# aluo-x/3D_SLN

Hardware: AMD Instinct MI355X
Metric: scene-graph VAE steps/sec + 256² diff-render fps, 1/2/4/8 MI355X (higher is better)
Workload: dtype f32; 1 GPU; BASELINE configs[1]: batch=64 scene graphs x (32 objects, 64 triples) per GPU, Sg2ScVAE train step at train.py defaults (embedding_dim=64, 5+5 GraphTripleConv, BatchNorm); O=2048, T=4096, hipgraph=True, distinct_batches_cycled=4, eps=N(0,1) drawn on the device inside the step, parallelism=dp1

## Files before the change

3d_sln_amd/_lib.py:

```python
from __future__ import annotations

import ctypes as C
import os

HERE = os.path.dirname(os.path.abspath(__file__))
LIB_PATH = os.path.join(HERE, "libsln_hip.so")

SLN_E = {-1: "SLN_E_BADARG", -2: "SLN_E_UNSUPPORTED", -3: "SLN_E_STATE", -4: "SLN_E_NOGPU", -5: "SLN_E_NOMEM", -6: "SLN_E_CAPTURE"}

c_f32p = C.c_void_p
c_i64p = C.c_void_p


class SlnError(RuntimeError):
    pass


class SlnVaeConfig(C.Structure):
    _fields_ = [(n, C.c_int) for n in (
        "embedding_dim", "gconv_num_layers", "recurrent", "batch_norm", "decoder_cat", "use_ae",
        "box_dim", "n_angle", "num_objs", "num_preds", "num_attrs", "no_attr")]


class SlnVaeUnit(C.Structure):
# ... 189 lines not shown
    "sln_debug_gemm_nt": (C.c_int, [C.POINTER(SlnDbgGemmNT), C.c_int, C.POINTER(C.c_int), C.c_void_p]),
    "sln_debug_gemm_tn": (C.c_int, [C.POINTER(SlnDbgGemmTN), C.c_int, C.c_int, C.c_void_p]),
    "sln_debug_gemm_nt_route": (C.c_int, [C.POINTER(SlnDbgGemmNT), C.POINTER(SlnDbgNTRoute)]),
    "sln_debug_gemm_nt_half": (C.c_int, [C.POINTER(SlnDbgGemmNT), C.c_int, C.c_void_p]),
    "sln_debug_gemm_nt_half_takes": (C.c_int, [C.POINTER(SlnDbgGemmNT)]),
    "sln_debug_gemm_sizes": (C.c_int, [C.POINTER(C.c_int), C.c_int]),
    "sln_debug_vae_csr": (C.c_int, [c_i64p, C.c_int, C.c_int, C.c_int, C.POINTER(SlnDbgCsr), C.c_void_p, C.c_void_p]),
    "sln_debug_vae_edge": (C.c_int, [C.POINTER(SlnDbgEdge), C.c_int, C.c_int, C.POINTER(C.c_int), C.c_void_p]),
    "sln_debug_vae_loss": (C.c_int, [C.POINTER(SlnDbgLoss), C.c_void_p]),
    "sln_debug_vae_tables": (C.c_int, [C.c_int, C.c_void_p, C.c_int, C.c_int, C.c_float, C.c_int, C.c_int, C.c_int, C.c_void_p]),
    "sln_debug_vae_embed": (C.c_int, [C.POINTER(SlnDbgEmbed), C.c_int, C.c_int, C.POINTER(C.c_int), C.c_void_p]),
    "sln_debug_vae_opt": (C.c_int, [C.POINTER(SlnDbgOpt), C.c_void_p]),
    "sln_debug_vae_sizes": (C.c_int, [C.POINTER(C.c_int), C.c_int]),
    "sln_debug_vae_leaf_launches": (C.c_int64, [C.c_void_p]),
    "sln_debug_vae_half_launches": (C.c_int64, [C.c_void_p]),
    "sln_project_faces": (C.c_int, [c_f32p, C.c_void_p, c_f32p, c_f32p, c_f32p, C.c_int, C.c_int, C.c_int, C.c_float, C.c_float, c_f32p, C.c_void_p]),
    "sln_project_faces_backward": (C.c_int, [c_f32p, C.c_void_p, c_f32p, c_f32p, c_f32p, C.c_int, C.c_int, C.c_int, C.c_float, C.c_float, c_f32p,
                                             c_f32p, C.c_void_p]),
    "sln_raster_workspace_bytes": (C.c_int64, [C.c_int, C.c_int]),
    "sln_raster_forward": (C.c_int, [c_f32p, C.c_int, C.c_int, C.c_int, C.c_float, C.c_float, C.c_void_p, C.c_void_p,
                                     c_f32p, c_f32p, C.c_void_p]),
    "sln_raster_forward_dual": (C.c_int, [c_f32p, C.c_int, C.c_int, C.c_int, C.c_float, C.c_float, C.c_float, C.c_void_p,
                                          C.c_void_p, c_f32p, c_f32p, C.c_void_p, c_f32p, c_f32p, C.c_void_p]),
    "sln_raster_texture_sample": (C.c_int, [c_f32p, c_f32p, C.c_void_p, c_f32p, c_f32p, C.c_int, C.c_int, C.c_int, C.c_int,
                                            C.c_float, c_f32p, C.c_void_p]),
    "sln_raster_backward_depth": (C.c_int, [c_f32p, C.c_void_p, c_f32p, c_f32p, c_f32p, C.c_int, C.c_int, C.c_int, c_f32p,
                                            C.c_void_p]),
    "sln_raster_backward_rgb": (C.c_int, [c_f32p, C.c_void_p, c_f32p, c_f32p, C.c_int, C.c_int, C.c_int, C.c_int, C.c_float,
                                          c_f32p, C.c_void_p]),
    "sln_raster_texture_sample_chw": (C.c_int, [c_f32p, c_f32p, C.c_void_p, c_f32p, c_f32p, C.c_int, C.c_int, C.c_int, C.c_int, C.c_int,
# ... 138 lines not shown
```

3d_sln_amd/csrc/sln_debug.h:

```cpp
#pragma once
#include "sln_common.h"
#include "sln_hip.h"

bool sln_dbg_bn(const SlnDbgBn& d, int coef, BnView& v);
long sln_vae_engine_leaf_launches(const SlnVae* h);
long sln_vae_engine_half_launches(const SlnVae* h);
```

3d_sln_amd/csrc/vae_debug.hip:

```cpp
#include <cstdint>
#include <cstring>
#include <vector>
#include "sln_debug.h"
#include "vae_multi.h"

namespace {

bool dbg_csr(const SlnDbgCsr& d, GraphCsr& g) {
  std::memset(&g, 0, sizeof(g));
  if (d.T < 0 || d.O < 1 || !d.deg || !d.invdeg || !d.rowptr || !d.cursor) return false;
  if (d.T > 0 && (!d.s || !d.p || !d.o || !d.ent)) return false;
  g.s = d.s; g.p = d.p; g.o = d.o; g.deg = d.deg; g.invdeg = d.invdeg; g.rowptr = d.rowptr; g.cursor = d.cursor; g.ent = d.ent;
  g.T = d.T; g.O = d.O;
  return true;
}

bool dbg_fwd_bn(const SlnDbgBn& d, int cols, BnView& v) {
  if (!sln_dbg_bn(d, SLN_COEF_FWD, v)) return false;
  return d.mode != SLN_BN_TRAIN || d.cstride >= cols;
}

enum { E_SCATTER_FWD = 0, E_SCATTER_BWD = 1, E_GATHER_BWD = 2, E_MASK_GSTATS = 3, E_BN_RELU = 4, E_ADD2 = 5 };

bool dbg_edge_ok(const SlnDbgEdge& d, GraphCsr& g, BnView& bn) {
// ... 150 lines not shown

extern "C" int sln_debug_vae_sizes(int* out, int max) {
  const int sz[7] = {(int)sizeof(SlnDbgCsr), (int)sizeof(SlnDbgEdge), (int)sizeof(SlnDbgLoss), (int)sizeof(SlnDbgBnEntry),
                     (int)sizeof(SlnDbgTranspose), (int)sizeof(SlnDbgOpt), (int)sizeof(SlnDbgEmbed)};
  for (int i = 0; out && i < 7 && i < max; ++i) out[i] = sz[i];
  return 7;
}

extern "C" int sln_debug_vae_csr(const int64_t* triples, int num_preds, int edges_only, int deg_is_zero, const SlnDbgCsr* desc, int* err,
                                 void* stream) {
  GraphCsr g;
  if (!desc || !dbg_csr(*desc, g) || (g.T > 0 && !triples) || (!edges_only && num_preds < 1)) return SLN_E_BADARG;
  return sln_launch_graph_prep(triples, g.T, g.O, edges_only ? 1 : num_preds, g, err, (hipStream_t)stream, edges_only ? 1 : 0, deg_is_zero ? 1 : 0);
}

extern "C" int sln_debug_vae_edge(const SlnDbgEdge* desc, int n, int multi, int* variant, void* stream) {
  if (!desc || n < 1 || n > 64 || (!multi && n != 1)) return SLN_E_BADARG;
  hipStream_t st = (hipStream_t)stream;
  std::vector<GraphCsr> g((size_t)n);
  std::vector<BnView> bn((size_t)n);
  for (int i = 0; i < n; ++i)
    if (desc[i].kind != desc[0].kind || !dbg_edge_ok(desc[i], g[(size_t)i], bn[(size_t)i])) return SLN_E_BADARG;
  if (variant) *variant = -1;
  if (!multi) return edge_single(desc[0], g[0], bn[0], st);
  if (sln_capturing(st)) return SLN_E_CAPTURE;
  switch (desc[0].kind) {
    case E_SCATTER_FWD: {
      std::vector<MScatterFwd> rooms((size_t)n);
      for (int i = 0; i < n; ++i) { const SlnDbgEdge& d = desc[i]; rooms[(size_t)i] = MScatterFwd{d.a, d.lda, d.H, d.D, bn[(size_t)i], g[(size_t)i], d.rows, d.out, 0, 0}; }
      return edge_multi(rooms, [](MScatterFwd& m) { return sln_plan_scatter_avg_fwd(m); }, [](const MScatterFwd* t, int R, int var, int gx, int gy, hipStream_t s) { return sln_launch_scatter_avg_fwd_multi(t, R, var, gx, gy, s); }, variant, st);
// ... 167 lines not shown
  for (int k = 0; k < d->calls && !r; ++k)
    r = d->kind == 0   ? sln_launch_adam(d->params, d->grads, d->m, d->v, (long)d->n, sc.p, d->total_loss, st)
        : d->kind == 1 ? sln_launch_randn(d->params, (long)d->n, sc.p, st)
                       : sln_launch_step_prologue(pro, st);
  const int rs = (int)hipStreamSynchronize(st);
  if (!r) r = rs;
  if (!r) r = (int)hipMemcpy(h.data(), sc.p, sizeof(AdamScalars), hipMemcpyDeviceToHost);
  if (sc.p) (void)hipFree(sc.p);
  if (r) return r;
  d->out_step = h[0].step; d->out_offset = h[0].rng_offset; d->out_bc1 = h[0].bc1; d->out_bc2 = h[0].bc2; d->out_skip = h[0].skip;
  if (h[0].adam_done != 0 || h[0].rng_done != 0) return SLN_E_STATE;
  return 0;
}

extern "C" int64_t sln_debug_vae_leaf_launches(const SlnVae* h) { return h ? (int64_t)sln_vae_engine_leaf_launches(h) : (int64_t)SLN_E_BADARG; }
extern "C" int64_t sln_debug_vae_half_launches(const SlnVae* h) { return h ? (int64_t)sln_vae_engine_half_launches(h) : (int64_t)SLN_E_BADARG; }
```

3d_sln_amd/csrc/vae_engine.hip:

```cpp
#include <cstddef>
#include <new>
#include <type_traits>
#include <utility>
#include <vector>
#include <cstring>
#include <cstdlib>

#include "../../include/sln_hip.h"
#include "sln_gemm.h"
#include "vae_kernels.h"
#include "vae_multi.h"
#include "sln_prof.h"

namespace {

enum { SK_DEC_ASSEMBLE = 0, SK_EMBED_GATHER, SK_NT, SK_SCATTER_FWD, SK_TN, SK_TN_FLUSH, SK_MASK_GSTATS, SK_ADD2, SK_EMBED_BWD,
       SK_SCATTER_BWD, SK_GATHER_BWD, SK_DEC_ASSEMBLE_BWD, SK_COPY2D };
struct RecStep {
  int kind = -1, epi = 0, idx64 = 0;
  GemmNTArgs nt; GemmTNArgs tn;
  MScatterFwd sf; MScatterBwd sb; MGatherBwd gb; MMaskGstats mg; MDecAssemble da; DecAssembleBwd dab; MEmbedGather eg; MEmbedBwd eb; MAdd2 a2;
};
struct Recorder { std::vector<RecStep> steps; };

// ... 216 lines not shown
    deferred.clear();
    return 0;
  }

  hipGraphExec_t graph_exec[4] = {nullptr, nullptr, nullptr, nullptr}; int graph_O[4] = {-1, -1, -1, -1}, graph_T[4] = {-1, -1, -1, -1};

  bool it_zero_in_prologue = false;
  bool it_prologue = false;
  bool it_fused_loss = false;
  bool it_one_flush = false;
  bool one_flush = true;
  bool it_merge_bn = false;
  bool no_merge = false;
  bool it_leaf = false;
  bool it_wt_prologue = false;
  bool leaf_merge = true;
  long leaf_launches = 0;
  int gemm_precision = 0;
  bool in_iteration = false;
  long half_launches = 0;
  bool gconv_only = false;
  int unit_of(int net, int l, int k) const { return (gconv_only ? 0 : 8) + (net * nmod + (cfg.recurrent ? 0 : l)) * 4 + k; }
  int unit_boxnet(int k) const { return 8 + 2 * nmod * 4 + k; }
  int unit_anglenet(int k) const { return 8 + 2 * nmod * 4 + 2 + k; }

  int bn_mode(const BnInst& b, bool training) const {
    if (b.unit < 0 || !units[b.unit].bn) return SLN_BN_NONE;
    return training ? SLN_BN_TRAIN : SLN_BN_EVAL;
  }
  BnView view(int inst, int col0, bool training) const {
    BnView v; std::memset(&v, 0, sizeof(v));
    v.eps = kBnEps; v.n_rows = 1.f; v.rn = 1.0; v.mode = SLN_BN_NONE;
// ... 358 lines not shown

int SlnVae::encoder_forward(bool training, hipStream_t st) {
  if (training && enc_stats_doubles && !bulk_zeroed) RET_IF(sln_zero_async(stats_base, enc_stats_doubles * sizeof(double), st));
  EncAssemble ea; std::memset(&ea, 0, sizeof(ea));
  ea.objs = batch.objs; ea.attrs = batch.attributes; ea.angles = batch.angles; ea.boxes = batch.boxes;
  ea.obj_emb = t.obj_emb_ec; ea.attr_emb = t.attr_emb_ec; ea.angle_emb = t.angle_emb; ea.wb = t.box_emb_w; ea.bb = t.box_emb_b;
  ea.O = O; ea.n_obj = n_obj_e; ea.n_attr = n_attr_e; ea.n_box = n_box_e; ea.n_angle = n_angle_e; ea.box_dim = cfg.box_dim;
  ea.x0 = X0e;
  if (it_prologue) {
    StepPrologue sp; std::memset(&sp, 0, sizeof(sp));
    sp.eps = draw_eps ? eps_buf : nullptr; sp.n_eps = (long)O * E; sp.scalars = scalars;
    sp.enc = ea; sp.pidx = g.p; sp.T = T;
    sp.pemb_ec = t.pred_emb_ec; sp.n_ec = Dec; sp.p0e = P0e;
    sp.pemb_dc = t.pred_emb_dc; sp.n_dc = Ddc; sp.p0d = P0d;
    if (it_zero_in_prologue) { sp.zero_ptr = zero_begin; sp.zero_bytes = (long)zero_bytes; }
    if (it_wt_prologue && !wt_fresh) { sp.tr_tab = tr_table_dev; sp.n_tr = n_tr; sp.tr_max_tiles = tr_max_tiles; }
    RET_IF(sln_launch_step_prologue(sp, st));
    if (sp.tr_tab) wt_fresh = true;
  } else {
    RET_IF(sln_launch_enc_assemble(ea, st));
    RET_IF(sln_launch_embed_gather_i32(g.p, t.pred_emb_ec, T, Dec, P0e, st));
  }
  for (int l = 0; l < L; ++l) RET_IF(gconv_forward(l, training, st));
  const Operand XL = layer_output(L - 1, training);
  const int W = 2 * E;
  begin_group();
  RET_IF(linear_fwd(XL, 0, hbA1, H, 0, O, bn_head[0], training, st));
  RET_IF(linear_fwd(XL, 4, haA1, H, 0, O, bn_head[2], training, st));
  RET_IF(end_group(st));
  begin_group();
// ... 204 lines not shown
    int maxc = 0;
    for (auto& bi : bns) maxc = bi.C > maxc ? bi.C : maxc;
    RET_IF(sln_launch_bn_param_grads(bn_table_dev, (int)bns.size(), maxc, cfg.recurrent ? 0 : 1, st));
  } else if (n_bn_enc > 0) {
    int maxc = 0;
    for (int i = 0; i < n_bn_enc; ++i) maxc = bns[i].C > maxc ? bns[i].C : maxc;
    RET_IF(sln_launch_bn_param_grads(bn_table_dev, n_bn_enc, maxc, cfg.recurrent ? 0 : 1, st));
  }
  RET_IF(flush_deferred(it_one_flush ? 2 : 1, st));
  return 0;
}

int SlnVae::train_iteration(const float* eps, int mode, hipStream_t st) {
  int r = 0;
  if (mode != TRAIN_ENCODER_BWD) {
    HIP_RET(hipMemsetAsync(t.flat_grads, 0, sizeof(float) * (size_t)t.n_flat, st));
    const bool no_merge = this->no_merge;
    it_prologue = it_fused_loss = !no_merge;
    it_zero_in_prologue = it_prologue && (reinterpret_cast<uintptr_t>(zero_begin) & 15) == 0 && (zero_bytes & 15) == 0;
    if (!it_zero_in_prologue) HIP_RET(hipMemsetAsync(zero_begin, 0, zero_bytes, st));
    bulk_zeroed = true;
    it_merge_bn = !no_merge && (mode == TRAIN_BACKWARD || mode == TRAIN_FULL);
    it_one_flush = one_flush && !tn_per_layer && (mode == TRAIN_BACKWARD || mode == TRAIN_FULL);
    it_leaf = it_merge_bn && dG[2] != nullptr && T > 0 && sln_vae_leaf_fits(leaf_args()) != 0;
    it_wt_prologue = it_prologue && leaf_merge && (mode == TRAIN_BACKWARD || mode == TRAIN_FULL);
    if (!it_prologue && draw_eps) r = sln_launch_randn(eps_buf, (long)O * E, scalars, st);
    in_iteration = true;
    if (!r) r = encoder_forward(step_training, st);
    if (!r) r = decoder_forward(nullptr, eps, step_training, st);
    in_iteration = false;
    if (!r) r = loss(boxes_pred, angles_pred, mu, logvar, true, st);
    if (!r && grad_guard && mode != TRAIN_FULL)
      r = (int)hipMemcpyAsync(grad_guard, losses + 3, sizeof(float), hipMemcpyDeviceToDevice, st);
    if (!r) r = decoder_backward(st);
    if (!r) r = sln_launch_latent_bwd(mu, logvar, eps, dz, &scalars->kl_weight, O, E, cfg.use_ae, dmu, dlv, st);
  }
  if (mode != TRAIN_UPTO_DECODER) {
    bulk_zeroed = true;
    if (!r) r = encoder_backward(st);
  }
  bulk_zeroed = false;
  it_prologue = it_fused_loss = it_merge_bn = it_zero_in_prologue = it_one_flush = it_leaf = it_wt_prologue = false;
  RET_IF(r);
  if (mode == TRAIN_FULL) {
    RET_IF(sln_launch_adam(t.flat_params, t.flat_grads, t.adam_m, t.adam_v, (long)t.n_flat, scalars, losses + 3, st));
    wt_fresh = false;
  }
  return 0;
}

long sln_vae_engine_leaf_launches(const SlnVae* h) { return h->leaf_launches; }
long sln_vae_engine_half_launches(const SlnVae* h) { return h->half_launches; }

extern "C" {

int sln_version(void) { return 1; }
const char* sln_build_arch(void) { return "gfx950"; }
int sln_device_ok(void) {
  int n = 0;
  if (hipGetDeviceCount(&n) != hipSuccess || n <= 0) return SLN_E_NOGPU;
  hipDeviceProp_t p;
  int dev = 0;
  if (hipGetDevice(&dev) != hipSuccess || hipGetDeviceProperties(&p, dev) != hipSuccess) return SLN_E_NOGPU;
  return std::strncmp(p.gcnArchName, "gfx950", 6) == 0 ? 0 : SLN_E_NOGPU;
}

static int cfg_check(const SlnVaeConfig* c) {
// ... 6 lines not shown
}

int sln_vae_num_units(const SlnVaeConfig* c) {
  if (cfg_check(c) != 0) return cfg_check(c);
  const int nmod = c->recurrent ? 1 : c->gconv_num_layers;
  return 8 + 2 * nmod * 4 + 4;
}

static int read_engine_options(SlnVae* h) {
  auto is = [](const char* name, char c) { const char* v = std::getenv(name); return v && v[0] == c; };
  h->use_group = !is("SLN_NO_GROUP", '1');
  h->no_merge = is("SLN_NO_MERGE", '1');
  h->tn_per_layer = is("SLN_TN_PER_LAYER", '1');
  h->one_flush = !is("SLN_TN_ONE_FLUSH", '0');
  h->leaf_merge = !is("SLN_LEAF_MERGE", '0');
  h->tn_slots = 3 * (2 * h->L + 8 > 16 ? 2 * h->L + 8 : 16);
  h->tn_groups_store = new (std::nothrow) SlnVae::TnGroup[2 * (size_t)h->tn_slots * 2];
  return h->tn_groups_store ? 0 : SLN_E_BADARG;
}

int sln_vae_create(const SlnVaeConfig* c, SlnVae** out) {
  if (!out) return SLN_E_BADARG;
  int r = cfg_check(c);
  if (r != 0) return r;
  SlnVae* h = new (std::nothrow) SlnVae();
  if (!h) return SLN_E_BADARG;
  h->cfg = *c;
  const int E = c->embedding_dim;
  h->E = E; h->H = 4 * E; h->L = c->gconv_num_layers; h->nmod = c->recurrent ? 1 : h->L;
  h->n_obj_e = c->no_attr ? E : E * 3 / 4; h->n_attr_e = c->no_attr ? 0 : E / 4; h->n_box_e = E * 3 / 4; h->n_angle_e = E / 4;
// ... 116 lines not shown
    for (auto& ly : h->layers)
      for (int k = 0; k < 4; ++k)
        if (ly.bn[k] >= 0) h->bns[ly.bn[k]].rows = k < 2 ? b->T : b->O;
    for (int s = 0; s < 6; ++s)
      if (h->bn_head[s] >= 0) h->bns[h->bn_head[s]].rows = b->O;
    if (!h->bn_table_live) {
      HIP_RET(hipStreamSynchronize(st));
      RET_IF(upload_bn_table(h));
      h->bn_table_live = true;
    }
    bool has_graph = false;
    for (int i = 0; i < 4; ++i) has_graph |= h->graph_exec[i] != nullptr;
    if (has_graph) HIP_RET(hipStreamSynchronize(st));
    h->drop_graphs();
  }
  RET_IF(sln_zero_async(h->err_flag, sizeof(int), st));
  StageBatch sb; std::memset(&sb, 0, sizeof(sb));
  sb.objs = b->objs; sb.attrs = b->attributes; sb.angles = b->angles; sb.boxes = b->boxes;
  sb.st_objs = h->st_objs; sb.st_attrs = h->st_attrs; sb.st_angles = h->st_angles; sb.st_boxes = h->st_boxes;
  sb.attrs32 = h->attrs32; sb.deg = h->g.deg; sb.err = h->err_flag;
  sb.O = b->O; sb.box_dim = h->cfg.box_dim; sb.n_objs = h->cfg.num_objs; sb.n_attrs = h->cfg.num_attrs; sb.n_angle = h->cfg.n_angle;
  RET_IF(sln_launch_stage_batch(sb, st));
  h->batch.objs = h->st_objs; h->batch.angles = h->st_angles; h->batch.attributes = h->st_attrs; h->batch.boxes = h->st_boxes;
  RET_IF(sln_launch_graph_prep(b->triples, b->T, b->O, h->cfg.num_preds, h->g, h->err_flag, st, 0, 1));
  h->batch_set = true; h->have_enc = h->have_dec = false;
  return 0;
}

int sln_vae_check_batch(SlnVae* h, void* stream) {
  if (!h || !h->batch_set) return SLN_E_STATE;
  int flag = 0;
  HIP_RET(hipMemcpyAsync(&flag, h->err_flag, sizeof(int), hipMemcpyDeviceToHost, (hipStream_t)stream));
  HIP_RET(hipStreamSynchronize((hipStream_t)stream));
  return flag ? SLN_E_BADARG : 0;
}

static int copy_out(float* dst, const float* src, size_t n, hipStream_t st) {
  if (!dst || dst == src) return 0;
  return (int)hipMemcpyAsync(dst, src, n * sizeof(float), hipMemcpyDeviceToDevice, st);
// ... 844 lines not shown
```

3d_sln_amd/csrc/vae_kernels.h:

```cpp
#pragma once
#include "sln_common.h"

struct GraphCsr {
  int* s;
  int* p;
  int* o;
  int* deg;
  float* invdeg;
  int* rowptr;
  int* cursor;
  int* ent;
  int T, O;
};
int sln_launch_graph_prep(const int64_t* triples, int T, int O, int num_preds, GraphCsr g, int* err_flag, hipStream_t st,
                          int edges_only = 0, int deg_is_zero = 0);
int sln_launch_bn_relu_apply(const float* x, int ld, int col0, int cols, int rows, BnView bn, float* out, int ldo, hipStream_t st);
struct StageBatch {
  const int64_t* objs; const int64_t* attrs; const int64_t* angles; const float* boxes;
  int64_t* st_objs; int64_t* st_attrs; int64_t* st_angles; float* st_boxes;
  int* attrs32; int* deg; int* err;
  int O, box_dim, n_objs, n_attrs, n_angle;
};
int sln_launch_stage_batch(const StageBatch& a, hipStream_t st);
int sln_launch_validate_ids(const int64_t* objs, const int64_t* attrs, const int64_t* angles, int O, int n_objs, int n_attrs,
                            int n_angle, int* err_flag, hipStream_t st);

int sln_launch_scatter_avg_fwd(const float* A2, int ld, int H, int D, BnView bn2, GraphCsr g, int O,
                               float* pooled, hipStream_t st);

int sln_launch_scatter_avg_bwd(const float* dM, const float* dP, int lddp, int dpcol0, const float* A2, int ld,
                               int H, int D, BnView bn2, GraphCsr g, int T, float* g2, double* gsums,
                               int cstride, hipStream_t st);

int sln_launch_gather_bwd(const float* dG, int ldg, int D, GraphCsr g, int O, const float* add1, int ldadd1,
                          const float* xprev, int ldx, BnView bn, int masked, float* out, int ldo,
                          double* gsums, int cstride, hipStream_t st);

int sln_launch_add2(const float* a, int lda, const float* b, int ldb, int rows, int cols, float* out, int ldo, hipStream_t st);
// ... 75 lines not shown
  int64_t step; float lr, beta1, beta2, eps; float kl_weight; float bc1, bc2; int skip, pad_;
  unsigned long long rng_seed, rng_offset; unsigned int rng_done, adam_done;
};
int sln_launch_adam(float* params, const float* grads, float* m, float* v, long n, AdamScalars* scalars, const float* total_loss,
                    hipStream_t st);

int sln_launch_randn(float* eps, long n, AdamScalars* scalars, hipStream_t st);

struct StepPrologue {
  float* eps; long n_eps; AdamScalars* scalars;
  EncAssemble enc;
  const int* pidx; int T;
  const float* pemb_ec; int n_ec; float* p0e;
  const float* pemb_dc; int n_dc; float* p0d;
  void* zero_ptr; long zero_bytes;
  const TransposeEntry* tr_tab; int n_tr, tr_max_tiles;
};
int sln_launch_step_prologue(const StepPrologue& a, hipStream_t st);

struct VaeLeaf {
  EncAssembleBwd enc;
  const int* pidx; int pred_rows, pred_table_rows;
  const float* d_pdc; int ld_pdc, col0_pdc, n_pdc; float* d_pred_dc;
  const float* d_pec; int ld_pec, col0_pec, n_pec; float* d_pred_ec;
  const int64_t* attr_idx; const float* d_attr; int ld_attr, col0_attr, n_attr_dc, attr_table_rows; float* d_attr_dc;
  const BnTableEntry* bn_tab; int bn_n, bn_max_c, bn_independent;
  int bn_update; float bn_momentum;
};
int sln_vae_leaf_fits(const VaeLeaf& a);
int sln_launch_vae_leaf(const VaeLeaf& a, hipStream_t st);
// ... 2 lines not shown
```

3d_sln_amd/csrc/vae_kernels.hip:

```cpp
#include <cstring>
#include "vae_kernels.h"
#include "sln_prof.h"

namespace {

constexpr int CB = 64;
constexpr int RL = 4;
constexpr int BOX_ROWS = 64;
constexpr int RB = 32;

__device__ __forceinline__ void commit_col_stats(float s1, float s2, bool valid, double* out, int cstride, int col) {
  __shared__ float red[2][RL][CB];
  red[0][threadIdx.y][threadIdx.x] = s1;
  red[1][threadIdx.y][threadIdx.x] = s2;
  __syncthreads();
  if (threadIdx.y == 0 && valid && out != nullptr) {
    float a = 0.f, b = 0.f;
#pragma unroll
    for (int i = 0; i < RL; ++i) { a += red[0][i][threadIdx.x]; b += red[1][i][threadIdx.x]; }
    atomicAdd(out + col, sln_qd((double)a, SLN_Q_BWD));
    atomicAdd(out + cstride + col, sln_qd((double)b, SLN_Q_BWD));
  }
}

// ... 806 lines not shown
    }
#pragma unroll
    for (int k = 0; k < 4; ++k)
      if (4 * q + k < n) eps[4 * q + k] = v[k];
  }
  __syncthreads();
  if (threadIdx.x == 0) {
    const unsigned int done = atomicAdd(&sc->rng_done, 1u);
    if (done == nblocks - 1) { sc->rng_done = 0; sc->rng_offset = off + 1; }
  }
}
__global__ __launch_bounds__(256) void randn_kernel(float* __restrict__ eps, long n, AdamScalars* sc) {
  randn_body(eps, n, sc, blockIdx.x, gridDim.x);
}

__global__ __launch_bounds__(256) void step_prologue_kernel(StepPrologue a, unsigned int b0, unsigned int b1, unsigned int b2, unsigned int b3,
                                                            unsigned int b4) {
  __shared__ float tile[32][33];
  const unsigned int b = blockIdx.x;
  if (b < b0) randn_body(a.eps, a.n_eps, a.scalars, b, b0);
  else if (b < b1) enc_assemble_body(a.enc, b - b0);
  else if (b < b2) embed_gather_body(a.pidx, a.pemb_ec, a.T, a.n_ec, a.p0e, b - b1);
  else if (b < b3) embed_gather_body(a.pidx, a.pemb_dc, a.T, a.n_dc, a.p0d, b - b2);
  else if (b < b4) {
    const long i = (long)(b - b3) * 256 + threadIdx.x;
    if (i * 16 < a.zero_bytes) reinterpret_cast<uint4*>(a.zero_ptr)[i] = make_uint4(0u, 0u, 0u, 0u);
  } else {
    const unsigned int q = b - b4;
    const TransposeEntry t = a.tr_tab[q / (unsigned int)a.tr_max_tiles];
    transpose_tile_body(t, (int)(q % (unsigned int)a.tr_max_tiles), tile);
  }
}

__global__ void bn_relu_apply_kernel(const float* __restrict__ x, int ld, int col0, int cols, long n, BnView bn,
                                     float* __restrict__ out, int ldo) {
  const long i = (long)blockIdx.x * blockDim.x + threadIdx.x;
  if (i >= n) return;
  const long r = i / cols; const int c = (int)(i % cols);
  float sc, sh;
  bn_fwd_coef(bn, c, sc, sh);
  out[r * ldo + c] = fmaxf(fmaf(sc, x[r * ld + col0 + c], sh), 0.f);
}

// ... 25 lines not shown
  const int i = blockIdx.x * blockDim.x + threadIdx.x;
  if (i >= a.O) return;
  const int64_t ob = a.objs[i], at = a.attrs[i], an = a.angles[i];
  a.st_objs[i] = ob; a.st_attrs[i] = at; a.st_angles[i] = an;
  a.attrs32[i] = (int)at;
  a.deg[i] = 0;
  for (int k = 0; k < a.box_dim; ++k) a.st_boxes[(size_t)i * a.box_dim + k] = a.boxes[(size_t)i * a.box_dim + k];
  if (ob < 0 || ob >= a.n_objs) atomicOr(a.err, 2);
  if (a.n_attrs > 0 && (at < 0 || at >= a.n_attrs)) atomicOr(a.err, 4);
  if (an < 0 || an >= a.n_angle) atomicOr(a.err, 8);
}

int sln_launch_stage_batch(const StageBatch& a, hipStream_t st) {
  if (a.O <= 0) return 0;
  hipLaunchKernelGGL(stage_batch_kernel, dim3(sln_cdiv(a.O, 256)), dim3(256), 0, st, a);
  SLN_CHECK_LAUNCH();
  return 0;
}

int sln_launch_validate_ids(const int64_t* objs, const int64_t* attrs, const int64_t* angles, int O, int n_objs, int n_attrs,
                            int n_angle, int* err_flag, hipStream_t st) {
  if (O <= 0) return 0;
  hipLaunchKernelGGL(validate_ids_kernel, dim3(sln_cdiv(O, 256)), dim3(256), 0, st, objs, attrs, angles, O, n_objs, n_attrs, n_angle,
                     err_flag);
  SLN_CHECK_LAUNCH();
  return 0;
}

int sln_launch_graph_prep(const int64_t* triples, int T, int O, int num_preds, GraphCsr g, int* err_flag, hipStream_t st,
                          int edges_only, int deg_is_zero) {
// ... 360 lines not shown

int sln_launch_randn(float* eps, long n, AdamScalars* scalars, hipStream_t st) {
  if (n <= 0) return 0;
  const long q = (n + 3) / 4;
  hipLaunchKernelGGL(randn_kernel, dim3((unsigned)((q + 255) / 256)), dim3(256), 0, st, eps, n, scalars);
  SLN_CHECK_LAUNCH();
  return 0;
}

int sln_launch_step_prologue(const StepPrologue& a, hipStream_t st) {
  auto blocks = [](long n) { return (unsigned int)((n + 255) / 256); };
  const unsigned int nr = a.eps ? blocks((a.n_eps + 3) / 4) : 0;
  const unsigned int ne = blocks((long)a.enc.O * (a.enc.n_obj + a.enc.n_attr + a.enc.n_box + a.enc.n_angle));
  const unsigned int n1 = blocks((long)a.T * a.n_ec), n2 = blocks((long)a.T * a.n_dc);
  const unsigned int nz = a.zero_ptr ? blocks(a.zero_bytes / 16) : 0;
  const unsigned int nt = (a.tr_tab && a.n_tr > 0 && a.tr_max_tiles > 0) ? (unsigned int)a.n_tr * (unsigned int)a.tr_max_tiles : 0;
  const unsigned int tot = nr + ne + n1 + n2 + nz + nt;
  if (tot == 0) return 0;
  hipLaunchKernelGGL(step_prologue_kernel, dim3(tot), dim3(256), 0, st, a, nr, nr + ne, nr + ne + n1, nr + ne + n1 + n2, nr + ne + n1 + n2 + nz);
  SLN_CHECK_LAUNCH();
  return 0;
}

struct LeafEmbedJob { const void* idx; const float* d; float* d_emb; int ld, col0, rows, n, table_rows, rpb; };
struct LeafArgs {
  AssembleBwdLds asmb;
  EncAssembleBwd box; int box_gx;
  LeafEmbedJob pdc, pec, attr;
  const BnTableEntry* bn_tab; int bn_n, bn_per_entry, bn_gx, rows_t, rows_o; float mom;
};
__global__ __launch_bounds__(256) void vae_leaf_kernel(unsigned int b0, unsigned int b1, unsigned int b2, unsigned int b3, unsigned int b4,
                                                       unsigned int b5, LeafArgs a) {
  extern __shared__ float tab[];
  const unsigned int b = blockIdx.x;
// ... 354 lines not shown
```

include/sln_hip.h:

```cpp
#ifndef SLN_HIP_H
#define SLN_HIP_H

#include <stdint.h>

#ifdef __cplusplus
extern "C" {
#endif

#define SLN_E_BADARG (-1)
#define SLN_E_UNSUPPORTED (-2)
#define SLN_E_STATE (-3)
#define SLN_E_NOGPU (-4)
#define SLN_E_NOMEM (-5)
#define SLN_E_CAPTURE (-6)

int sln_version(void);
const char* sln_build_arch(void);
int sln_device_ok(void);


typedef struct SlnVaeConfig {
  int embedding_dim;
  int gconv_num_layers;
  int recurrent;
// ... 220 lines not shown
  int kind, O, n_obj, n_attr, n_box, n_angle, box_dim, n_z, use_ae, z_in_x0, rows_obj, rows_attr, rows_angle, ld, col0, n, table_rows,
      T, n2, pad_;
} SlnDbgEmbed;
int sln_debug_vae_embed(const SlnDbgEmbed* desc, int n, int multi, int* variant, void* stream);
typedef struct SlnDbgOpt {
  float* params; const float* grads; float* m; float* v; const float* total_loss; const SlnDbgEmbed* pro;
  int64_t n, step;
  uint64_t seed, offset;
  float lr, beta1, beta2, eps;
  int kind, calls;
  int64_t out_step; uint64_t out_offset; float out_bc1, out_bc2; int out_skip, pad_;
} SlnDbgOpt;
int sln_debug_vae_opt(SlnDbgOpt* desc, void* stream);
int sln_debug_vae_sizes(int* out, int max);
int64_t sln_debug_vae_leaf_launches(const SlnVae* h);
int64_t sln_debug_vae_half_launches(const SlnVae* h);


int sln_project_faces(const float* vertices, const int32_t* faces, const float* K, const float* R, const float* t, int B, int V, int F,
                      float orig_size, float eps, float* faces_xyz, void* stream);
int sln_project_faces_backward(const float* vertices, const int32_t* faces, const float* K, const float* R, const float* t, int B, int V,
                               int F, float orig_size, float eps, const float* grad_faces_xyz, float* grad_vertices, void* stream);
int64_t sln_raster_workspace_bytes(int B, int F);
int sln_raster_forward(const float* faces, int B, int F, int image_size, float near, float far, void* workspace,
                       int32_t* face_index, float* weight, float* depth, void* stream);
int sln_raster_forward_dual(const float* faces, int B, int F, int image_size, float near_a, float near_b, float far,
                            void* workspace, int32_t* fi_a, float* w_a, float* d_a, int32_t* fi_b, float* w_b,
                            float* d_b, void* stream);
int sln_raster_texture_sample(const float* faces, const float* textures, const int32_t* face_index, const float* weight,
                              const float* depth, int B, int F, int image_size, int texture_size, float eps, float* rgb,
// ... 199 lines not shown
```

Before: 35500 graphs/s (scene-graph VAE fwd+loss+bwd+Adam).

## Fuse batch staging and CSR graph prep into one kernel; merge grad clear into prologue

```diff
diff --git a/3d_sln_amd/_lib.py b/3d_sln_amd/_lib.py
--- a/3d_sln_amd/_lib.py
+++ b/3d_sln_amd/_lib.py
@@ -227,6 +227,9 @@
     "sln_debug_vae_sizes": (C.c_int, [C.POINTER(C.c_int), C.c_int]),
     "sln_debug_vae_leaf_launches": (C.c_int64, [C.c_void_p]),
     "sln_debug_vae_half_launches": (C.c_int64, [C.c_void_p]),
+    "sln_debug_vae_bind": (C.c_int, [c_i64p, C.c_int, C.POINTER(SlnDbgCsr), C.POINTER(SlnDbgEmbed), C.c_void_p]),
+    "sln_debug_vae_bind_fits": (C.c_int, [C.c_int, C.c_int]),
+    "sln_debug_vae_bind_launches": (C.c_int64, [C.c_void_p]),
     "sln_project_faces": (C.c_int, [c_f32p, C.c_void_p, c_f32p, c_f32p, c_f32p, C.c_int, C.c_int, C.c_int, C.c_float, C.c_float, c_f32p, C.c_void_p]),
     "sln_project_faces_backward": (C.c_int, [c_f32p, C.c_void_p, c_f32p, c_f32p, c_f32p, C.c_int, C.c_int, C.c_int, C.c_float, C.c_float, c_f32p,
                                              c_f32p, C.c_void_p]),
diff --git a/3d_sln_amd/csrc/sln_debug.h b/3d_sln_amd/csrc/sln_debug.h
--- a/3d_sln_amd/csrc/sln_debug.h
+++ b/3d_sln_amd/csrc/sln_debug.h
@@ -5,3 +5,4 @@
 bool sln_dbg_bn(const SlnDbgBn& d, int coef, BnView& v);
 long sln_vae_engine_leaf_launches(const SlnVae* h);
 long sln_vae_engine_half_launches(const SlnVae* h);
+long sln_vae_engine_bind_merged(const SlnVae* h);
diff --git a/3d_sln_amd/csrc/vae_debug.hip b/3d_sln_amd/csrc/vae_debug.hip
--- a/3d_sln_amd/csrc/vae_debug.hip
+++ b/3d_sln_amd/csrc/vae_debug.hip
@@ -188,6 +188,20 @@
   return sln_launch_graph_prep(triples, g.T, g.O, edges_only ? 1 : num_preds, g, err, (hipStream_t)stream, edges_only ? 1 : 0, deg_is_zero ? 1 : 0);
 }
 
+extern "C" int sln_debug_vae_bind_fits(int O, int T) { return sln_vae_bind_fits(O, T); }
+
+extern "C" int sln_debug_vae_bind(const int64_t* triples, int num_preds, const SlnDbgCsr* desc, const SlnDbgEmbed* stage, void* stream) {
+  GraphCsr g;
+  if (!desc || !stage || !dbg_csr(*desc, g) || (g.T > 0 && !triples) || num_preds < 1) return SLN_E_BADARG;
+  const SlnDbgEmbed& d = *stage;
+  if (d.O != g.O || !d.objs || !d.attrs || !d.angles || !d.boxes || !d.st_objs || !d.st_attrs || !d.st_angles || !d.st_boxes || !d.attrs32 ||
+      !d.err || d.box_dim < 1 || d.rows_obj < 0 || d.rows_attr < 0 || d.rows_angle < 0)
+    return SLN_E_BADARG;
+  if (!sln_vae_bind_fits(g.O, g.T)) return SLN_E_UNSUPPORTED;
+  return sln_launch_vae_bind(StageBatch{d.objs, d.attrs, d.angles, d.boxes, d.st_objs, d.st_attrs, d.st_angles, d.st_boxes, d.attrs32, g.deg, d.err,
+                                        d.O, d.box_dim, d.rows_obj, d.rows_attr, d.rows_angle}, triples, num_preds, g, (hipStream_t)stream);
+}
+
 extern "C" int sln_debug_vae_edge(const SlnDbgEdge* desc, int n, int multi, int* variant, void* stream) {
   if (!desc || n < 1 || n > 64 || (!multi && n != 1)) return SLN_E_BADARG;
   hipStream_t st = (hipStream_t)stream;
@@ -385,4 +399,5 @@
 }
 
 extern "C" int64_t sln_debug_vae_leaf_launches(const SlnVae* h) { return h ? (int64_t)sln_vae_engine_leaf_launches(h) : (int64_t)SLN_E_BADARG; }
+extern "C" int64_t sln_debug_vae_bind_launches(const SlnVae* h) { return h ? (int64_t)sln_vae_engine_bind_merged(h) : (int64_t)SLN_E_BADARG; }
 extern "C" int64_t sln_debug_vae_half_launches(const SlnVae* h) { return h ? (int64_t)sln_vae_engine_half_launches(h) : (int64_t)SLN_E_BADARG; }
diff --git a/3d_sln_amd/csrc/vae_engine.hip b/3d_sln_amd/csrc/vae_engine.hip
--- a/3d_sln_amd/csrc/vae_engine.hip
+++ b/3d_sln_amd/csrc/vae_engine.hip
@@ -254,8 +254,12 @@
   bool no_merge = false;
   bool it_leaf = false;
   bool it_wt_prologue = false;
+  bool it_grads_in_prologue = false;
   bool leaf_merge = true;
   long leaf_launches = 0;
+  bool bind_merge = true;
+  bool grad_clear_merge = true;
+  bool bind_merged = false;
   int gemm_precision = 0;
   bool in_iteration = false;
   long half_launches = 0;
@@ -644,6 +648,7 @@
     sp.pemb_ec = t.pred_emb_ec; sp.n_ec = Dec; sp.p0e = P0e;
     sp.pemb_dc = t.pred_emb_dc; sp.n_dc = Ddc; sp.p0d = P0d;
     if (it_zero_in_prologue) { sp.zero_ptr = zero_begin; sp.zero_bytes = (long)zero_bytes; }
+    if (it_grads_in_prologue) { sp.grad_ptr = t.flat_grads; sp.grad_bytes = (long)(sizeof(float) * (size_t)t.n_flat); }
     if (it_wt_prologue && !wt_fresh) { sp.tr_tab = tr_table_dev; sp.n_tr = n_tr; sp.tr_max_tiles = tr_max_tiles; }
     RET_IF(sln_launch_step_prologue(sp, st));
     if (sp.tr_tab) wt_fresh = true;
@@ -878,9 +883,12 @@
 int SlnVae::train_iteration(const float* eps, int mode, hipStream_t st) {
   int r = 0;
   if (mode != TRAIN_ENCODER_BWD) {
-    HIP_RET(hipMemsetAsync(t.flat_grads, 0, sizeof(float) * (size_t)t.n_flat, st));
     const bool no_merge = this->no_merge;
     it_prologue = it_fused_loss = !no_merge;
+    const size_t grad_bytes = sizeof(float) * (size_t)t.n_flat;
+    it_grads_in_prologue = it_prologue && grad_clear_merge && (mode == TRAIN_BACKWARD || mode == TRAIN_FULL) &&
+                           (reinterpret_cast<uintptr_t>(t.flat_grads) & 15) == 0 && (grad_bytes & 15) == 0;
+    if (!it_grads_in_prologue) HIP_RET(hipMemsetAsync(t.flat_grads, 0, grad_bytes, st));
     it_zero_in_prologue = it_prologue && (reinterpret_cast<uintptr_t>(zero_begin) & 15) == 0 && (zero_bytes & 15) == 0;
     if (!it_zero_in_prologue) HIP_RET(hipMemsetAsync(zero_begin, 0, zero_bytes, st));
     bulk_zeroed = true;
@@ -904,7 +912,7 @@
     if (!r) r = encoder_backward(st);
   }
   bulk_zeroed = false;
-  it_prologue = it_fused_loss = it_merge_bn = it_zero_in_prologue = it_one_flush = it_leaf = it_wt_prologue = false;
+  it_prologue = it_fused_loss = it_merge_bn = it_zero_in_prologue = it_one_flush = it_leaf = it_wt_prologue = it_grads_in_prologue = false;
   RET_IF(r);
   if (mode == TRAIN_FULL) {
     RET_IF(sln_launch_adam(t.flat_params, t.flat_grads, t.adam_m, t.adam_v, (long)t.n_flat, scalars, losses + 3, st));
@@ -915,6 +923,7 @@
 
 long sln_vae_engine_leaf_launches(const SlnVae* h) { return h->leaf_launches; }
 long sln_vae_engine_half_launches(const SlnVae* h) { return h->half_launches; }
+long sln_vae_engine_bind_merged(const SlnVae* h) { return h->batch_set ? (h->bind_merged ? 1 : 0) : -1; }
 
 extern "C" {
 
@@ -951,6 +960,8 @@
   h->tn_per_layer = is("SLN_TN_PER_LAYER", '1');
   h->one_flush = !is("SLN_TN_ONE_FLUSH", '0');
   h->leaf_merge = !is("SLN_LEAF_MERGE", '0');
+  h->bind_merge = !is("SLN_BIND_MERGE", '0');
+  h->grad_clear_merge = !is("SLN_GRAD_CLEAR_MERGE", '0');
   h->tn_slots = 3 * (2 * h->L + 8 > 16 ? 2 * h->L + 8 : 16);
   h->tn_groups_store = new (std::nothrow) SlnVae::TnGroup[2 * (size_t)h->tn_slots * 2];
   return h->tn_groups_store ? 0 : SLN_E_BADARG;
@@ -1097,15 +1108,20 @@
     if (has_graph) HIP_RET(hipStreamSynchronize(st));
     h->drop_graphs();
   }
-  RET_IF(sln_zero_async(h->err_flag, sizeof(int), st));
   StageBatch sb; std::memset(&sb, 0, sizeof(sb));
   sb.objs = b->objs; sb.attrs = b->attributes; sb.angles = b->angles; sb.boxes = b->boxes;
   sb.st_objs = h->st_objs; sb.st_attrs = h->st_attrs; sb.st_angles = h->st_angles; sb.st_boxes = h->st_boxes;
   sb.attrs32 = h->attrs32; sb.deg = h->g.deg; sb.err = h->err_flag;
   sb.O = b->O; sb.box_dim = h->cfg.box_dim; sb.n_objs = h->cfg.num_objs; sb.n_attrs = h->cfg.num_attrs; sb.n_angle = h->cfg.n_angle;
-  RET_IF(sln_launch_stage_batch(sb, st));
   h->batch.objs = h->st_objs; h->batch.angles = h->st_angles; h->batch.attributes = h->st_attrs; h->batch.boxes = h->st_boxes;
-  RET_IF(sln_launch_graph_prep(b->triples, b->T, b->O, h->cfg.num_preds, h->g, h->err_flag, st, 0, 1));
+  h->bind_merged = h->bind_merge && sln_vae_bind_fits(b->O, b->T) != 0;
+  if (h->bind_merged) {
+    RET_IF(sln_launch_vae_bind(sb, b->triples, h->cfg.num_preds, h->g, st));
+  } else {
+    RET_IF(sln_zero_async(h->err_flag, sizeof(int), st));
+    RET_IF(sln_launch_stage_batch(sb, st));
+    RET_IF(sln_launch_graph_prep(b->triples, b->T, b->O, h->cfg.num_preds, h->g, h->err_flag, st, 0, 1));
+  }
   h->batch_set = true; h->have_enc = h->have_dec = false;
   return 0;
 }
diff --git a/3d_sln_amd/csrc/vae_kernels.h b/3d_sln_amd/csrc/vae_kernels.h
--- a/3d_sln_amd/csrc/vae_kernels.h
+++ b/3d_sln_amd/csrc/vae_kernels.h
@@ -22,6 +22,8 @@
   int O, box_dim, n_objs, n_attrs, n_angle;
 };
 int sln_launch_stage_batch(const StageBatch& a, hipStream_t st);
+int sln_vae_bind_fits(int O, int T);
+int sln_launch_vae_bind(const StageBatch& a, const int64_t* triples, int num_preds, GraphCsr g, hipStream_t st);
 int sln_launch_validate_ids(const int64_t* objs, const int64_t* attrs, const int64_t* angles, int O, int n_objs, int n_attrs,
                             int n_angle, int* err_flag, hipStream_t st);
 
@@ -127,6 +129,7 @@
   const float* pemb_ec; int n_ec; float* p0e;
   const float* pemb_dc; int n_dc; float* p0d;
   void* zero_ptr; long zero_bytes;
+  float* grad_ptr; long grad_bytes;
   const TransposeEntry* tr_tab; int n_tr, tr_max_tiles;
 };
 int sln_launch_step_prologue(const StepPrologue& a, hipStream_t st);
diff --git a/3d_sln_amd/csrc/vae_kernels.hip b/3d_sln_amd/csrc/vae_kernels.hip
--- a/3d_sln_amd/csrc/vae_kernels.hip
+++ b/3d_sln_amd/csrc/vae_kernels.hip
@@ -844,8 +844,9 @@
   randn_body(eps, n, sc, blockIdx.x, gridDim.x);
 }
 
+constexpr int PRO_GRAD_VEC = 16;
 __global__ __launch_bounds__(256) void step_prologue_kernel(StepPrologue a, unsigned int b0, unsigned int b1, unsigned int b2, unsigned int b3,
-                                                            unsigned int b4) {
+                                                            unsigned int b4, unsigned int b5) {
   __shared__ float tile[32][33];
   const unsigned int b = blockIdx.x;
   if (b < b0) randn_body(a.eps, a.n_eps, a.scalars, b, b0);
@@ -855,8 +856,16 @@
   else if (b < b4) {
     const long i = (long)(b - b3) * 256 + threadIdx.x;
     if (i * 16 < a.zero_bytes) reinterpret_cast<uint4*>(a.zero_ptr)[i] = make_uint4(0u, 0u, 0u, 0u);
+  } else if (b < b5) {
+    const long n = a.grad_bytes / 16;
+    float4* g = reinterpret_cast<float4*>(a.grad_ptr);
+#pragma unroll 4
+    for (int k = 0; k < PRO_GRAD_VEC; ++k) {
+      const long i = ((long)(b - b4) * PRO_GRAD_VEC + k) * 256 + threadIdx.x;
+      if (i < n) g[i] = make_float4(0.f, 0.f, 0.f, 0.f);
+    }
   } else {
-    const unsigned int q = b - b4;
+    const unsigned int q = b - b5;
     const TransposeEntry t = a.tr_tab[q / (unsigned int)a.tr_max_tiles];
     transpose_tile_body(t, (int)(q % (unsigned int)a.tr_max_tiles), tile);
   }
@@ -912,6 +921,165 @@
 int sln_launch_stage_batch(const StageBatch& a, hipStream_t st) {
   if (a.O <= 0) return 0;
   hipLaunchKernelGGL(stage_batch_kernel, dim3(sln_cdiv(a.O, 256)), dim3(256), 0, st, a);
+  SLN_CHECK_LAUNCH();
+  return 0;
+}
+
+constexpr int BIND_THREADS = 1024;
+constexpr int BIND_FIXED_INTS = 32;
+constexpr int BIND_KEEP = 8;
+constexpr size_t BIND_LDS_MAX = 160 * 1024;
+
+__device__ __forceinline__ bool bind_triple(const int64_t* __restrict__ tri, int t, int O, int num_preds, int& s, int& p, int& o) {
+  const int64_t s64 = tri[3 * (size_t)t], p64 = tri[3 * (size_t)t + 1], o64 = tri[3 * (size_t)t + 2];
+  const bool ok = !(s64 < 0 || s64 >= O || o64 < 0 || o64 >= O || p64 < 0 || p64 >= num_preds);
+  s = ok ? (int)s64 : 0; p = ok ? (int)p64 : 0; o = ok ? (int)o64 : 0;
+  return ok;
+}
+
+__device__ __forceinline__ void bind_place(const int* ent, const int* rp, int node, int e, int* __restrict__ out) {
+  const int b = rp[node], n = rp[node + 1] - b;
+  int rank = 0, j = 0;
+  for (; j + 8 <= n; j += 8) {
+    int v[8];
+#pragma unroll
+    for (int q = 0; q < 8; ++q) v[q] = ent[b + j + q];
+#pragma unroll
+    for (int q = 0; q < 8; ++q) rank += v[q] < e ? 1 : 0;
+  }
+  for (; j < n; ++j) rank += ent[b + j] < e ? 1 : 0;
+  out[b + rank] = e;
+}
+
+__global__ __launch_bounds__(BIND_THREADS) void vae_bind_kernel(StageBatch a, const int64_t* __restrict__ tri, int T, int num_preds, GraphCsr g) {
+  extern __shared__ int bind_lds[];
+  const int O = a.O, tid = threadIdx.x;
+  if (blockIdx.x > 0) {
+    const int i = (blockIdx.x - 1) * BIND_THREADS + tid;
+    if (i < O) {
+      const int64_t at = a.attrs[i];
+      a.st_objs[i] = a.objs[i]; a.st_attrs[i] = at; a.st_angles[i] = a.angles[i];
+      a.attrs32[i] = (int)at;
+      for (int k = 0; k < a.box_dim; ++k) a.st_boxes[(size_t)i * a.box_dim + k] = a.boxes[(size_t)i * a.box_dim + k];
+    }
+    if (i < T) {
+      int s, p, o;
+      bind_triple(tri, i, O, num_preds, s, p, o);
+      g.s[i] = s; g.p[i] = p; g.o[i] = o;
+    }
+    return;
+  }
+  int* wsum = bind_lds;
+  int* errw = bind_lds + 16;
+  int* cnt = bind_lds + BIND_FIXED_INTS;
+  int* rp = cnt + O;
+  int* ent = rp + O + 1;
+  int pk[BIND_KEEP];
+  int bad = 0;
+#pragma unroll
+  for (int k = 0; k < BIND_KEEP; ++k) {
+    const int t = tid + k * BIND_THREADS;
+    pk[k] = -1;
+    if (t < T) {
+      int s, p, o;
+      if (!bind_triple(tri, t, O, num_preds, s, p, o)) bad |= 1;
+      pk[k] = s | (o << 16);
+    }
+  }
+  for (int i = tid; i < O; i += BIND_THREADS) {
+    const int64_t ob = a.objs[i], at = a.attrs[i], an = a.angles[i];
+    if (ob < 0 || ob >= a.n_objs) bad |= 2;
+    if (a.n_attrs > 0 && (at < 0 || at >= a.n_attrs)) bad |= 4;
+    if (an < 0 || an >= a.n_angle) bad |= 8;
+  }
+  for (int i = tid; i < O; i += BIND_THREADS) cnt[i] = 0;
+  if (tid == 0) *errw = 0;
+  __syncthreads();
+#pragma unroll
+  for (int k = 0; k < BIND_KEEP; ++k)
+    if (pk[k] != -1) {
+      atomicAdd(cnt + (pk[k] & 0xffff), 1);
+      atomicAdd(cnt + (int)((unsigned int)pk[k] >> 16), 1);
+    }
+  for (int t = tid + BIND_KEEP * BIND_THREADS; t < T; t += BIND_THREADS) {
+    int s, p, o;
+    if (!bind_triple(tri, t, O, num_preds, s, p, o)) bad |= 1;
+    atomicAdd(cnt + s, 1);
+    atomicAdd(cnt + o, 1);
+  }
+  if (bad) atomicOr(errw, bad);
+  __syncthreads();
+  const int K = (O + BIND_THREADS - 1) / BIND_THREADS;
+  const int lo = tid * K < O ? tid * K : O, hi = lo + K < O ? lo + K : O;
+  int sum = 0;
+  for (int i = lo; i < hi; ++i) sum += cnt[i];
+  const int lane = tid & 63, wave = tid >> 6;
+  int incl = sum;
+#pragma unroll
+  for (int off = 1; off < 64; off <<= 1) {
+    const int v = __shfl_up(incl, off, 64);
+    if (lane >= off) incl += v;
+  }
+  if (lane == 63) wsum[wave] = incl;
+  __syncthreads();
+  int run = incl - sum;
+  for (int w = 0; w < wave; ++w) run += wsum[w];
+  for (int i = lo; i < hi; ++i) { rp[i] = run; run += cnt[i]; }
+  if (tid == BIND_THREADS - 1) rp[O] = run;
+  __syncthreads();
+  for (int i = tid; i < O; i += BIND_THREADS) {
+    const int d = cnt[i];
+    g.deg[i] = d; g.rowptr[i] = rp[i];
+    g.invdeg[i] = 1.0f / (float)(d > 1 ? d : 1);
+  }
+  if (tid == 0) { g.rowptr[O] = rp[O]; *a.err = *errw; }
+  __syncthreads();
+#pragma unroll
+  for (int k = 0; k < BIND_KEEP; ++k)
+    if (pk[k] != -1) {
+      const int t = tid + k * BIND_THREADS, s = pk[k] & 0xffff, o = (int)((unsigned int)pk[k] >> 16);
+      ent[rp[s] + atomicSub(cnt + s, 1) - 1] = t;
+      ent[rp[o] + atomicSub(cnt + o, 1) - 1] = t + T;
+    }
+  for (int t = tid + BIND_KEEP * BIND_THREADS; t < T; t += BIND_THREADS) {
+    int s, p, o;
+    bind_triple(tri, t, O, num_preds, s, p, o);
+    ent[rp[s] + atomicSub(cnt + s, 1) - 1] = t;
+    ent[rp[o] + atomicSub(cnt + o, 1) - 1] = t + T;
+  }
+  __syncthreads();
+#pragma unroll
+  for (int k = 0; k < BIND_KEEP; ++k)
+    if (pk[k] != -1) {
+      const int t = tid + k * BIND_THREADS;
+      bind_place(ent, rp, pk[k] & 0xffff, t, g.ent);
+      bind_place(ent, rp, (int)((unsigned int)pk[k] >> 16), t + T, g.ent);
+    }
+  for (int t = tid + BIND_KEEP * BIND_THREADS; t < T; t += BIND_THREADS) {
+    int s, p, o;
+    bind_triple(tri, t, O, num_preds, s, p, o);
+    bind_place(ent, rp, s, t, g.ent);
+    bind_place(ent, rp, o, t + T, g.ent);
+  }
+}
+
+static size_t bind_lds_bytes(long O, long T) { return sizeof(int) * (size_t)(BIND_FIXED_INTS + 2 * O + 1 + 2 * T); }
+
+int sln_vae_bind_fits(int O, int T) { return (O >= 1 && T >= 0 && bind_lds_bytes(O, T) <= BIND_LDS_MAX) ? 1 : 0; }
+
+int sln_launch_vae_bind(const StageBatch& a, const int64_t* triples, int num_preds, GraphCsr g, hipStream_t st) {
+  if (!sln_vae_bind_fits(g.O, g.T) || a.O != g.O || !a.err || (g.T > 0 && !triples)) return -1;
+  const size_t lds = bind_lds_bytes(g.O, g.T);
+  if (lds > 48 * 1024) {
+    static bool raised = false;
+    if (!raised) {
+      hipError_t e = hipFuncSetAttribute(reinterpret_cast<const void*>(&vae_bind_kernel), hipFuncAttributeMaxDynamicSharedMemorySize, (int)BIND_LDS_MAX);
+      if (e != hipSuccess) return (int)e;
+      raised = true;
+    }
+  }
+  const int most = g.O > g.T ? g.O : g.T;
+  hipLaunchKernelGGL(vae_bind_kernel, dim3(1 + sln_cdiv(most, BIND_THREADS)), dim3(BIND_THREADS), lds, st, a, triples, g.T, num_preds, g);
   SLN_CHECK_LAUNCH();
   return 0;
 }
@@ -1302,10 +1470,12 @@
   const unsigned int ne = blocks((long)a.enc.O * (a.enc.n_obj + a.enc.n_attr + a.enc.n_box + a.enc.n_angle));
   const unsigned int n1 = blocks((long)a.T * a.n_ec), n2 = blocks((long)a.T * a.n_dc);
   const unsigned int nz = a.zero_ptr ? blocks(a.zero_bytes / 16) : 0;
+  const unsigned int ng = (a.grad_ptr && a.grad_bytes > 0) ? (unsigned int)((a.grad_bytes / 16 + 256L * PRO_GRAD_VEC - 1) / (256L * PRO_GRAD_VEC)) : 0;
   const unsigned int nt = (a.tr_tab && a.n_tr > 0 && a.tr_max_tiles > 0) ? (unsigned int)a.n_tr * (unsigned int)a.tr_max_tiles : 0;
-  const unsigned int tot = nr + ne + n1 + n2 + nz + nt;
+  const unsigned int tot = nr + ne + n1 + n2 + nz + ng + nt;
   if (tot == 0) return 0;
-  hipLaunchKernelGGL(step_prologue_kernel, dim3(tot), dim3(256), 0, st, a, nr, nr + ne, nr + ne + n1, nr + ne + n1 + n2, nr + ne + n1 + n2 + nz);
+  hipLaunchKernelGGL(step_prologue_kernel, dim3(tot), dim3(256), 0, st, a, nr, nr + ne, nr + ne + n1, nr + ne + n1 + n2, nr + ne + n1 + n2 + nz,
+                     nr + ne + n1 + n2 + nz + ng);
   SLN_CHECK_LAUNCH();
   return 0;
 }
diff --git a/include/sln_hip.h b/include/sln_hip.h
--- a/include/sln_hip.h
+++ b/include/sln_hip.h
@@ -258,6 +258,9 @@
 int sln_debug_vae_opt(SlnDbgOpt* desc, void* stream);
 int sln_debug_vae_sizes(int* out, int max);
 int64_t sln_debug_vae_leaf_launches(const SlnVae* h);
+int sln_debug_vae_bind(const int64_t* triples, int num_preds, const SlnDbgCsr* g, const SlnDbgEmbed* stage, void* stream);
+int sln_debug_vae_bind_fits(int O, int T);
+int64_t sln_debug_vae_bind_launches(const SlnVae* h);
 int64_t sln_debug_vae_half_launches(const SlnVae* h);
 
 
```

Measured after the change: 35630 graphs/s (scene-graph VAE fwd+loss+bwd+Adam) (median of 6 runs). Within noise of the previous version (+0.4%).
